# gnlpfjh/Scalable-E3-GNN

Measured on AMD Instinct MI355X. Metric: particles/sec (octree build + SEGNN fwd), 1M pts l_max=2, 1/2/4/8 MI355X, higher is better.
Workload: dtype f32; 1 GPU; 1000000 particles/GPU uniform in unit box, radius graph k~24 (E=23519616), SEGNN l_max=2 4 layers H=32 f32 storage; particles_per_gpu=1000000, edges_per_gpu=23519616, hidden=32, layers=4, lmax=2, parallelism=single GPU

## Files before the change

### scalable-e3-gnn_amd/csrc/e3_msg_ws.hip

```cpp
#include "e3_msg_plan.h"
#include "cg_tables.h"

#include <algorithm>
#include <type_traits>

#ifndef E3_WS_STAMP
#define E3_WS_STAMP 0
#endif

namespace e3 {
#include "e3_tp_mfma_core.h"
#include "e3_msg_common.h"

#if E3_WS_STAMP
__device__ unsigned long long g_ws_stamps[8][4];
__device__ unsigned long long g_ws_tp[8][8];
#define WS_TPMARK(i) { if (tpm) { const uint32_t t_ = (uint32_t)__builtin_readcyclecounter(); tpm[i] += t_ - tpm0; tpm0 = t_; } }
#define WS_TPPIN(v) asm volatile("" : "+v"(v));
#else
#define WS_TPMARK(i)
#define WS_TPPIN(v)
#endif

template <int LMAX, int TT, bool IO16>
struct Ws {
  using G = MsgGeom<LMAX, TT>;
  static_assert(TT == 2 && (LMAX == 1 || LMAX == 2), "instantiated for H = 32, l_max = 1 / 2");
  static constexpr int H = G::H, D = G::D, NS = G::NS, UD = G::UD;
  static constexpr int ES = IO16 ? 2 : 4;
  static constexpr int NC = (LMAX + 1) * (LMAX + 1);
  static constexpr int NFR = NC + LMAX;
  static constexpr int FRB = IO16 ? 1024 : 2048;
  static constexpr int frag(int l, int a) { return l * l + a; }
  static constexpr int frag_ff(int l) { return NC + l - 1; }
  static constexpr int GA_ROW = (NC - 1) * H * ES;
  static constexpr int GA_STRIDE = GA_ROW + 16;
  static constexpr int GA_BYTES = 16 * GA_STRIDE;
  static constexpr int GB_ROW = H * ES;
  static constexpr int GB_BYTES = 16 * GB_ROW;
  static constexpr int G_BYTES = GA_BYTES + GB_BYTES;
  static constexpr int RS = D + 4;
  static constexpr int U_ROW = UD * 4;
  static constexpr int U_PIECES = (U_ROW + 1023) / 1024, U_LAST = (U_ROW - (U_PIECES - 1) * 1024) / 16;
  static_assert(U_ROW % 16 == 0, "pre-mix rows are copied in 16-byte units");
  static constexpr int o_tab = 0;
  static constexpr int o_tinfo = (o_tab + (2 * NS * 16 + G::WD) * 4 + 15) / 16 * 16;
  static constexpr int o_ids = o_tinfo + 4 * 32;
  static constexpr int o_idok = o_ids + 4 * 128;
  static constexpr int o_pos = o_idok + 16;
  static constexpr int o_hmx = o_pos + 2 * 512;
  static constexpr int o_srow = o_hmx + 2 * 128;
  static constexpr int z_y = 0, z_112 = 12, z_121 = 28, z_211 = 40, z_222 = 56, ZT = LMAX == 2 ? 84 : 12;
  static constexpr int o_zt = o_srow + 2 * 64;
  static constexpr int o_init = o_zt + 2 * 16 * ZT * 4;
  static constexpr bool PRE = !IO16;
  static constexpr int P_AROW = (NC - 1) * 128;
  static constexpr int P_ASTRIDE = P_AROW + 32;
  static constexpr int P_ALANES = P_AROW / 16;
  static constexpr int o_pz = 16 * P_ASTRIDE, o_pf = o_pz + 2048;
  static constexpr int P_IMG = o_pf + LMAX * 2048;
  static constexpr int p_asrc(int lane) { return 128 + 16 * lane; }
  static constexpr int p_alds(int row, int lane) { return row * P_ASTRIDE + 16 * lane; }
  static constexpr int p_zrow(int piece, int lane) { return 8 * piece + (lane & 7); }
  static constexpr int p_zsrc(int lane) { return 64 * ((lane >> 5) & 1) + 16 * (2 * ((lane >> 4) & 1) + ((lane >> 3) & 1)); }
  static constexpr int p_zlds(int piece, int lane) { return o_pz + 1024 * piece + 16 * lane; }
  static constexpr int p_zpos(int lane) {
    return 1024 * ((lane & 15) >> 3) + 256 * (lane >> 5) + 128 * ((lane >> 4) & 1) + 16 * (lane & 7);
  }
  static constexpr int p_abase(int lane) { return (lane & 15) * P_ASTRIDE + 16 * (lane >> 4); }
  static constexpr int p_zbase(int lane) { return o_pz + p_zpos(lane); }
  static constexpr bool p_on_a(int fr) { return fr >= 1 && fr < NC; }
  static constexpr int p_off(int fr, int half) {
    return p_on_a(fr) ? 128 * (fr - 1) + 64 * half : (fr == 0 ? 0 : 2048 * (1 + fr - NC)) + 512 * half;
  }
  static constexpr int p_read(int fr, int half, int lane) { return (p_on_a(fr) ? p_abase(lane) : p_zbase(lane)) + p_off(fr, half); }
  static constexpr int o_g = o_init + G::T(0) * 1024;
  static constexpr int o_b1 = o_g + (PRE ? 2 * P_IMG : G_BYTES);
  static constexpr int o_b2 = o_b1 + (PRE ? 0 : NFR * FRB);
  static constexpr int o_o = o_b2 + NFR * FRB;
  static constexpr int o_u = o_o + 16 * RS * 4;
  static constexpr int total = o_u + 4 * U_ROW;
  static_assert(total <= 160 * 1024, "LDS image exceeds the CU");
};

template <int LMAX, int TT>
struct WsImageCheck {
  using L = Ws<LMAX, TT, false>;
  static constexpr int NU = L::o_pf / 16;
  static constexpr int group_lane(int grp, int i) {
    const int base = 32 * (grp >> 1), odd = grp & 1;
    const int k = odd ? (i < 8 ? 4 + i : (i < 12 ? 16 + (i - 8) : 28 + (i - 12))) : (i < 4 ? i : (i < 8 ? 12 + (i - 4) : 20 + (i - 8)));
    return base + k;
  }
  static constexpr bool run() {
    int owner_row[NU] = {}, owner_unit[NU] = {}, count[NU] = {};
    for (int r = 0; r < 16; ++r)
      for (int l = 0; l < L::P_ALANES; ++l) {
        const int u = L::p_alds(r, l) / 16;
        if (L::p_alds(r, l) % 16 || u < 0 || u >= NU) return false;
        ++count[u]; owner_row[u] = r; owner_unit[u] = L::p_asrc(l) / 16;
      }
    for (int p = 0; p < 2; ++p)
      for (int l = 0; l < 64; ++l) {
        const int u = L::p_zlds(p, l) / 16;
        if (u < 0 || u >= NU) return false;
        ++count[u]; owner_row[u] = L::p_zrow(p, l); owner_unit[u] = L::p_zsrc(l) / 16;
      }
    int written = 0;
    for (int u = 0; u < NU; ++u) {
      if (count[u] > 1) return false;
      written += count[u];
    }
    if (written != 16 * MsgSplit<LMAX>::UNITS) return false;
    for (int fr = 0; fr < L::NC; ++fr)
      for (int half = 0; half < 2; ++half) {
        for (int lane = 0; lane < 64; ++lane) {
          const int a = L::p_read(fr, half, lane), u = a / 16;
          if (a % 16 || u < 0 || u >= NU || count[u] != 1) return false;
          if (owner_row[u] != (lane & 15) || owner_unit[u] != MsgSplit<LMAX>::unit(fr, half, lane >> 4)) return false;
        }
      }
    for (int fr = 0; fr < L::NFR; ++fr)
      for (int half = 0; half < 2; ++half)
        for (int grp = 0; grp < 4; ++grp) {
          bool seen[16] = {};
          for (int i = 0; i < 16; ++i) {
            const int a = L::p_read(fr, half, group_lane(grp, i));
            if (a < 0 || a + 16 > L::P_IMG) return false;
            const int slot = (a % 256) / 16;
            if (seen[slot]) return false;
            seen[slot] = true;
          }
        }
    for (int fr = L::NC; fr < L::NFR; ++fr)
      for (int half = 0; half < 2; ++half)
        for (int lane = 0; lane < 64; ++lane)
          for (int l2 = lane + 1; l2 < 64; ++l2)
            if (L::p_read(fr, half, lane) == L::p_read(fr, half, l2) || L::p_read(fr, half, lane) < L::o_pf) return false;
    return true;
  }
};
static_assert(WsImageCheck<2, 2>::run() && WsImageCheck<1, 2>::run(), "pre-split image: coverage, read map or bank conflicts");

struct TileInfo { int e0, n, n0, node0, node1, sl0, sl1; };

__device__ __forceinline__ void dma16(const void* gsrc, uint32_t lds_dst) {
  uint32_t keep;
  asm volatile("s_mov_b32 %0, m0\n\ts_mov_b32 m0, %2\n\ts_nop 0\n\tglobal_load_lds_dwordx4 %1, off\n\ts_mov_b32 m0, %0"
               : "=&s"(keep) : "v"(gsrc), "s"(lds_dst) : "memory");
}
__device__ __forceinline__ void dma16_stream(const void* gsrc, uint32_t lds_dst) {
  uint32_t keep;
  asm volatile("s_mov_b32 %0, m0\n\ts_mov_b32 m0, %2\n\ts_nop 0\n\tglobal_load_lds_dwordx4 %1, off nt\n\ts_mov_b32 m0, %0"
               : "=&s"(keep) : "v"(gsrc), "s"(lds_dst) : "memory");
}
__device__ __forceinline__ void dma4(const void* gsrc, uint32_t lds_dst) {
  uint32_t keep;
  asm volatile("s_mov_b32 %0, m0\n\ts_mov_b32 m0, %2\n\ts_nop 0\n\tglobal_load_lds_dword %1, off\n\ts_mov_b32 m0, %0"
               : "=&s"(keep) : "v"(gsrc), "s"(lds_dst) : "memory");
}
__device__ __forceinline__ void ws_wait_vm0() { asm volatile("s_waitcnt vmcnt(0)" ::: "memory"); }
__device__ __forceinline__ void ws_barrier() { asm volatile("s_waitcnt lgkmcnt(0)\n\ts_barrier" ::: "memory"); }
__device__ __forceinline__ int sgpr(int v) { return __builtin_amdgcn_readfirstlane(v); }
__device__ __forceinline__ void split2_f16_scaled(const float v0, const float v1, const float s, uint32_t& hi, uint32_t& lo) {
  uint32_t h, l;
  asm("v_fma_mixlo_f16 %0, %1, %2, 0 op_sel_hi:[0,0,0]" : "=v"(h) : "v"(s), "v"(v0));
  asm("v_fma_mixhi_f16 %0, %1, %2, 0 op_sel_hi:[0,0,0]" : "+v"(h) : "v"(s), "v"(v1));
  asm("v_fma_mixlo_f16 %0, %1, %2, -%3 op_sel:[0,0,0] op_sel_hi:[0,0,1]" : "=v"(l) : "v"(s), "v"(v0), "v"(h));
  asm("v_fma_mixhi_f16 %0, %1, %2, -%3 op_sel:[0,0,1] op_sel_hi:[0,0,1]" : "+v"(l) : "v"(s), "v"(v1), "v"(h));
  hi = h; lo = l;
}
template <bool IO16>
__device__ __forceinline__ void ws_put4(unsigned char* dst, const float (&f)[4], const float s) {
  if constexpr (IO16) {
    const uint32_t a = __builtin_bit_cast(uint32_t, __builtin_convertvector(f32x2_t{f[0], f[1]}, bf16x2_t));
    const uint32_t b = __builtin_bit_cast(uint32_t, __builtin_convertvector(f32x2_t{f[2], f[3]}, bf16x2_t));
    *reinterpret_cast<uint2*>(dst) = uint2{a, b};
  } else {
    uint32_t h0, l0, h1, l1;
    split2_f16_scaled(f[0], f[1], s, h0, l0);
    split2_f16_scaled(f[2], f[3], s, h1, l1);
    *reinterpret_cast<uint2*>(dst) = uint2{h0, h1};
    *reinterpret_cast<uint2*>(dst + 1024) = uint2{l0, l1};
  }
}
template <int HI>
__device__ __forceinline__ float fma_mix_h(const float z, const uint32_t pair, const float acc) {
  float d;
  if constexpr (HI) asm("v_fma_mix_f32 %0, %1, %2, %3 op_sel:[0,1,0] op_sel_hi:[0,1,0]" : "=v"(d) : "v"(z), "v"(pair), "v"(acc));
  else asm("v_fma_mix_f32 %0, %1, %2, %3 op_sel:[0,0,0] op_sel_hi:[0,1,0]" : "=v"(d) : "v"(z), "v"(pair), "v"(acc));
  return d;
}
__device__ __forceinline__ uint32_t u4_word(const uint4& v, const int i) { return i == 0 ? v.x : i == 1 ? v.y : i == 2 ? v.z : v.w; }
template <class F>
__device__ __forceinline__ void sfor3(F&& f) {
  f(std::integral_constant<int, 0>{}); f(std::integral_constant<int, 1>{}); f(std::integral_constant<int, 2>{});
}

template <int LMAX, int TT, int ROLE>
struct Own {
  using G = MsgGeom<LMAX, TT>;
  static constexpr int t = ROLE & 1;
  static constexpr int LV = ROLE < 2 ? LMAX : LMAX - 1;
  static constexpr int tG = LV > 0 ? TT * LV + t : -1;
  static constexpr int tS = ROLE >= 2 ? t : -1;
  static constexpr int sl3(int s) { return s == 0 ? LV : 0; }
  static constexpr int stile(int s) { return s == 0 ? t : s == 1 ? tG : tS; }
  static constexpr bool shas(int s) { return s == 0 ? LV > 0 : stile(s) >= 0; }
  static constexpr bool has(int s, int l1, int l2) { return shas(s) && G::ok(l1, l2, sl3(s)); }
  static constexpr int widx(int s, int l1, int l2) {
    int n = 0;
    for (int ss = 0; ss < 3; ++ss)
      for (int a = 0; a <= LMAX; ++a)
        for (int b = 0; b <= LMAX; ++b) {
          if (ss == s && a == l1 && b == l2) return has(ss, a, b) ? n : -1;
          if (has(ss, a, b)) ++n;
        }
    return n;
  }
  static constexpr int NW = widx(3, 0, 0);
};

template <int NW>
struct RoleW { uint4 h[NW], l[NW]; };

template <int LMAX, int TT, int ROLE, bool IO16>
__device__ __forceinline__ void ws_load_w(const float* packed, const int prod , const int lane,
                                          RoleW<Own<LMAX, TT, ROLE>::NW>& w) {
  using G = MsgGeom<LMAX, TT>;
  using O = Own<LMAX, TT, ROLE>;
  const unsigned char* base = reinterpret_cast<const unsigned char*>(packed + G::o_w) + (size_t)prod * G::nblk() * 2048 + lane * 16;
  auto one = [&](auto stag, auto atag, auto btag) {
    constexpr int s = decltype(stag)::value, l1 = decltype(atag)::value, l2 = decltype(btag)::value;
    if constexpr (l1 <= LMAX && l2 <= LMAX && O::has(s, l1, l2)) {
      constexpr int i = O::widx(s, l1, l2), blk = G::blk(l1, l2, O::sl3(s)) + O::stile(s);
      w.h[i] = *reinterpret_cast<const uint4*>(base + (size_t)blk * 2048);
      if constexpr (!IO16) w.l[i] = *reinterpret_cast<const uint4*>(base + (size_t)blk * 2048 + 1024);
      else w.l[i] = uint4{0, 0, 0, 0};
    }
  };
  using I0 = std::integral_constant<int, 0>; using I1 = std::integral_constant<int, 1>; using I2 = std::integral_constant<int, 2>;
  auto slot = [&](auto stag) {
    one(stag, I0{}, I0{}); one(stag, I0{}, I1{}); one(stag, I0{}, I2{});
    one(stag, I1{}, I0{}); one(stag, I1{}, I1{}); one(stag, I1{}, I2{});
    one(stag, I2{}, I0{}); one(stag, I2{}, I1{}); one(stag, I2{}, I2{});
  };
  slot(I0{}); slot(I1{}); slot(I2{});
}

constexpr int kWsPF = 2;
constexpr int kWsXrot = 2;
constexpr int kWsPKT = 15;
#ifndef WS_PKZ
#define WS_PKZ 11
#endif
constexpr int kWsPrio = 0;
template <int LMAX>
struct TpItems {
  static constexpr int N = (LMAX + 1) * (LMAX + 1) + LMAX;
  static constexpr int len(int l) { return 2 * l + 1 + (l > 0 ? 1 : 0); }
  static constexpr int start(int l) { int n = 0; for (int k = LMAX; k > l; --k) n += len(k); return n; }
  static constexpr int l1(int i) { int l = LMAX; while (l > 0 && i >= start(l) + len(l)) --l; return l; }
  static constexpr int a(int i) { const int l = l1(i), k = i - start(l); return k < 2 * l + 1 ? k : -1; }
  static constexpr bool first(int i) { return i == start(l1(i)); }
};

template <int LMAX, int TT, int ROLE, bool FIRST, bool IO16>
struct TpRun {
  using G = MsgGeom<LMAX, TT>;
  using O = Own<LMAX, TT, ROLE>;
  using L = Ws<LMAX, TT, IO16>;
  using IT = TpItems<LMAX>;
  static constexpr int LV = O::LV, t = O::t, tG = O::tG, tS = O::tS;
  static constexpr bool SC = tG >= 0 || tS >= 0;

  static constexpr bool PIMG = FIRST && L::PRE;
  const RoleW<O::NW>& w;
  const unsigned char* bfr;
  const unsigned char* bfz;
  int lane;
  const float* zt;
  const float* urow;
  const float* wd;
  const f32x4* init;
  f32x4 (&accV)[5];
  f32x4& accG;
  f32x4& accS;
  float dsc;
  uint4 bh[kWsPF + 1], bl[kWsPF + 1];
  f32x4 uV[3][3][5];
  f32x4 wdV;
  f32x4 yv[3];
  f32x4 zq[3][3][7];
#if E3_WS_STAMP
  uint32_t* tpm = nullptr;
  uint32_t tpm0 = 0;
#endif
  static constexpr int zoff(int l1, int l2) {
    return (l1 == 1 && l2 == 1 && LV == 2) ? L::z_112 : (l1 == 1 && l2 == 2 && LV == 1) ? L::z_121
         : (l1 == 2 && l2 == 1 && LV == 1) ? L::z_211 : (l1 == 2 && l2 == 2 && LV == 2) ? L::z_222 : -1;
  }
  __device__ __forceinline__ float yy(const int i) const { return yv[i >> 2][i & 3]; }

  template <int I>
  __device__ __forceinline__ void request() {
    if constexpr (I < IT::N) {
      constexpr int L1 = IT::l1(I), a = IT::a(I), slot = I % (kWsPF + 1);
      constexpr int fr = a >= 0 ? L::frag(L1, a) : L::frag_ff(L1);
      if constexpr (a >= 0 || SC) {
        if constexpr (PIMG) {
          const unsigned char* b = bfr;
          if constexpr (!L::p_on_a(fr)) {
            int l = lane;
            asm volatile("" : "+v"(l));
            b = bfz + L::p_zbase(l);
          }
          bh[slot] = *reinterpret_cast<const uint4*>(b + L::p_off(fr, 0));
          bl[slot] = *reinterpret_cast<const uint4*>(b + L::p_off(fr, 1));
        } else {
          bh[slot] = *reinterpret_cast<const uint4*>(bfr + fr * L::FRB);
          if constexpr (!IO16) bl[slot] = *reinterpret_cast<const uint4*>(bfr + fr * L::FRB + 1024);
          else bl[slot] = uint4{0, 0, 0, 0};
        }
      }
      const f32x4 zero4 = {0.f, 0.f, 0.f, 0.f};
      if constexpr (a >= 0) {
        sfor3([&](auto l2tag) {
          constexpr int L2 = decltype(l2tag)::value;
          if constexpr (LV > 0 && G::ok(L1, L2, LV)) {
            if constexpr (FIRST) uV[L1][L2][a] = *reinterpret_cast<const f32x4*>(urow + G::uoff(L1, L2, LV) + (a * G::T(LV) + t) * 16);
            else uV[L1][L2][a] = zero4;
            if constexpr (a == 0 && zoff(L1, L2) >= 0) {
              constexpr int NZ = ((2 * L1 + 1) * (2 * LV + 1) + 3) / 4;
#pragma unroll
              for (int q = 0; q < NZ; ++q) zq[L1][L2][q] = *reinterpret_cast<const f32x4*>(zt + zoff(L1, L2) + 4 * q);
            }
          }
        });
        if constexpr (L1 == 0 && FIRST && LV > 0) wdV = *reinterpret_cast<const f32x4*>(wd + G::wdoff(LV) + t * 16);
      }
    }
  }

  template <int I>
  __device__ __forceinline__ void compute() {
    constexpr int L1 = IT::l1(I), a = IT::a(I), slot = I % (kWsPF + 1);
    const uint4 xh = bh[slot], xl = bl[slot];
    if constexpr (a >= 0) {
      if constexpr (L1 == 0 && FIRST && LV > 0) {
        uV[0][LV][0] = __builtin_elementwise_fma(wdV, f32x4{dsc, dsc, dsc, dsc}, uV[0][LV][0]);
      }
      sfor3([&](auto l2tag) {
        constexpr int L2 = decltype(l2tag)::value;
        if constexpr (LV > 0 && G::ok(L1, L2, LV)) {
          constexpr int i = O::widx(0, L1, L2);
          uV[L1][L2][a] = mma3<IO16>(w.h[i], w.l[i], xh, xl, uV[L1][L2][a]);
        }
      });
      if constexpr (L1 == 0) {
        if constexpr (tG >= 0) accG = mma3<IO16>(w.h[O::widx(1, 0, 0)], w.l[O::widx(1, 0, 0)], xh, xl, accG);
        if constexpr (tS >= 0) accS = mma3<IO16>(w.h[O::widx(2, 0, 0)], w.l[O::widx(2, 0, 0)], xh, xl, accS);
      }
    } else if constexpr (SC) {
      if constexpr (tG >= 0) accG = mma3<IO16>(w.h[O::widx(1, L1, L1)], w.l[O::widx(1, L1, L1)], xh, xl, accG);
      if constexpr (tS >= 0) accS = mma3<IO16>(w.h[O::widx(2, L1, L1)], w.l[O::widx(2, L1, L1)], xh, xl, accS);
    }
  }

  template <int L1>
  __device__ __forceinline__ void fold() {
    constexpr int D1 = 2 * L1 + 1;
    sfor3([&](auto l2tag) {
      constexpr int L2 = decltype(l2tag)::value;
      if constexpr (LV > 0 && G::ok(L1, L2, LV)) {
        constexpr int D3 = 2 * LV + 1;
        if constexpr (zoff(L1, L2) >= 0) {
#pragma unroll
          for (int c = 0; c < D3; ++c)
#pragma unroll
            for (int aa = 0; aa < D1; ++aa)
              if (z_nonzero<L1, L2, LV>(aa, c)) {
                const float z = zq[L1][L2][(aa * D3 + c) >> 2][(aa * D3 + c) & 3];
                constexpr int zi = (L1 == 1 && L2 == 1) ? 0 : (L1 == 1 && L2 == 2) ? 1 : (L1 == 2 && L2 == 1) ? 2 : 3;
                if constexpr (!IO16 && (kWsPKT & 1) && ((WS_PKZ >> zi) & 1)) {
                  accV[c] = __builtin_elementwise_fma(uV[L1][L2][aa], f32x4{z, z, z, z}, accV[c]);
                } else {
#pragma unroll
                  for (int r = 0; r < 4; ++r) accV[c][r] = __builtin_fmaf(uV[L1][L2][aa][r], z, accV[c][r]);
                }
              }
        } else {
          float y9[9];
#pragma unroll
          for (int i = 0; i < 9; ++i) y9[i] = yy(i);
          float zz[D1][D3];
          make_z<L1, L2, LV>(y9, zz);
#pragma unroll
          for (int c = 0; c < D3; ++c)
#pragma unroll
            for (int aa = 0; aa < D1; ++aa)
              if (z_nonzero<L1, L2, LV>(aa, c)) {
                if constexpr (!IO16 && (kWsPKT & 2)) {
                  accV[c] = __builtin_elementwise_fma(uV[L1][L2][aa], f32x4{zz[aa][c], zz[aa][c], zz[aa][c], zz[aa][c]}, accV[c]);
                } else {
#pragma unroll
                  for (int r = 0; r < 4; ++r) accV[c][r] = __builtin_fmaf(uV[L1][L2][aa][r], zz[aa][c], accV[c][r]);
                }
              }
        }
      }
    });
  }

  template <int I>
  __device__ __forceinline__ void step() {
    request<I + kWsPF>();
    __builtin_amdgcn_sched_barrier(0);
    compute<I>();
    if constexpr (IT::first(I) && IT::l1(I) < LMAX) fold<IT::l1(I) + 1>();
    if constexpr (I + 1 < IT::N && IT::first(I + 1)) { WS_TPMARK(1 + LMAX - IT::l1(I)) }
    if constexpr (I + 1 < IT::N) step<I + 1>();
    else { pin_products(); WS_TPMARK(1 + LMAX) fold<0>(); pin_folds(); WS_TPMARK(2 + LMAX) }
  }
  __device__ __forceinline__ void pin_products() {
    if constexpr (LV > 0) { WS_TPPIN(uV[0][LV][0]) }
    WS_TPPIN(accG) WS_TPPIN(accS)
  }
  __device__ __forceinline__ void pin_folds() {
#pragma unroll
    for (int c = 0; c < 2 * LV + 1; ++c) { WS_TPPIN(accV[c]) }
  }

  __device__ __forceinline__ void run() {
    const f32x4 zero4 = {0.f, 0.f, 0.f, 0.f};
#pragma unroll
    for (int c = 0; c < 5; ++c) accV[c] = zero4;
#pragma unroll
    for (int q = 0; q < 3; ++q) yv[q] = *reinterpret_cast<const f32x4*>(zt + L::z_y + 4 * q);
    accG = zero4; accS = zero4;
    if constexpr (FIRST) {
      if constexpr (tG >= 0) accG = init[64 * tG];
      if constexpr (tS >= 0) accS = init[64 * tS];
    }
    request<0>();
    if constexpr (kWsPF >= 2) request<1>();
    if constexpr (kWsPF >= 3) request<2>();
    static_assert(kWsPF >= 1 && kWsPF <= 3, "prefetch distance");
    __builtin_amdgcn_sched_barrier(0);
    dsc = yv[2][1];
    WS_TPMARK(0)
    step<0>();
  }
};

template <int LMAX, int TT, int ROLE, bool FIRST, bool IO16>
__device__ __forceinline__ void ws_tp(const RoleW<Own<LMAX, TT, ROLE>::NW>& w, const unsigned char* bfr,
                                      const unsigned char* bfz, const int lane, const float* zt,
                                      const float* urow, const float* wd, const f32x4* init,
                                      f32x4 (&accV)[5], f32x4& accG, f32x4& accS, float (&y)[10], uint32_t* tpmarks = nullptr) {
  TpRun<LMAX, TT, ROLE, FIRST, IO16> r{w, bfr, bfz, lane, zt, urow, wd, init, accV, accG, accS};
#if E3_WS_STAMP
  r.tpm = tpmarks;
  r.tpm0 = (uint32_t)__builtin_readcyclecounter();
#endif
  r.run();
#pragma unroll
  for (int i = 0; i < 10; ++i) y[i] = r.yy(i);
}

template <class BOX>
struct WsArgsT {
  const void* h; int64_t ldh;
  const float4* pos4; const int32_t* src; const int32_t* dst; int64_t E;
  const float* packed; const float* U; const void* split; const float* hmax; const float* in_scale; float* out; int64_t ldo;
  int chunk;
  float* part; int* part_node; uint32_t* amax; int chunks_per_xcd;
  BOX box;
};
using WsArgs = WsArgsT<PbcBox>;

template <int LMAX, int TT, bool IO16, int W, int PBC>
__device__ __forceinline__ void ws_run(const WsArgsT<typename PbcArg<PBC>::type>& A, unsigned char* smem) {
  using G = MsgGeom<LMAX, TT>;
  using L = Ws<LMAX, TT, IO16>;
  constexpr int H = G::H, D = G::D, ES = L::ES;
  constexpr bool TEAM1 = W >= 4;
  constexpr int ROLE = W & 3;
  constexpr int SX = TEAM1 ? -1 : ((W + kWsXrot) & 3);
  constexpr int ITB = SX < 0 ? 0 : L::PRE ? (SX == 2 ? 4 : 0) : 2 * SX;
  constexpr int ITE0 = SX < 0 ? 0 : L::PRE ? (SX == 1 ? 4 : (SX == 2 ? 6 : 0)) : (SX <= 2 ? 2 * SX + 2 : 2 * SX);
  constexpr int ITE = ITE0 < G::T(0) ? ITE0 : G::T(0);
  constexpr int SY = TEAM1 ? (W & 3) : -1;
  using O = Own<LMAX, TT, ROLE>;
  using I0 = std::integral_constant<int, 0>; using I1 = std::integral_constant<int, 1>; using I2 = std::integral_constant<int, 2>;
  const int lane = threadIdx.x & 63, j = lane & 15, g = lane >> 4;
  const uint32_t lds0 = (uint32_t)(uintptr_t)smem;
  const float* n1tab = reinterpret_cast<const float*>(smem + L::o_tab);
  const float* n2tab = n1tab + G::NS * 16;
  const float* wdtab = n2tab + G::NS * 16;
  const float xs = (!IO16 && A.in_scale) ? A.in_scale[0] : 1.0f;
  const float bwx = A.packed[6] * ((!IO16 && A.in_scale) ? A.in_scale[1] : 1.0f);
  const char* hb = reinterpret_cast<const char*>(A.h);

  auto tinfo = [&](const int tile) -> TileInfo {
    TileInfo ti = {0, 0, 0, -1, -1, 0, 0};
    if (tile >= 0) {
      const int4* p = reinterpret_cast<const int4*>(smem + L::o_tinfo + (tile & 3) * 32);
      const int4 a = p[0], b = p[1];
      ti.e0 = sgpr(a.x); ti.n = sgpr(a.y); ti.n0 = sgpr(a.z); ti.node0 = sgpr(a.w);
      ti.node1 = sgpr(b.x); ti.sl0 = sgpr(b.y); ti.sl1 = sgpr(b.z);
    }
    return ti;
  };

  RoleW<O::NW> w;
  ws_load_w<LMAX, TT, ROLE, IO16>(A.packed, TEAM1 ? 1 : 0, lane, w);
  wait_vm0();
  f32x4 nrS = {0.f, 0.f, 0.f, 0.f}, nrG = {0.f, 0.f, 0.f, 0.f}, nrV[5];
  {
    const f32x4* ntq = reinterpret_cast<const f32x4*>(TEAM1 ? n2tab : n1tab) + g;
    if constexpr (O::tS >= 0) nrS = ntq[4 * O::tS];
#pragma unroll
    for (int c = 0; c < 5; ++c) nrV[c] = f32x4{0.f, 0.f, 0.f, 0.f};
    if constexpr (O::LV > 0) {
      nrG = ntq[4 * O::tG];
#pragma unroll
      for (int c = 0; c < 2 * O::LV + 1; ++c) nrV[c] = ntq[4 * (G::slot0(O::LV) + (2 * O::LV + 1) * O::t + c)];
    }
  }

  const int Ei = (int)A.E;
  const int per_xcd = (int)(gridDim.x >> 3), wg_idx = (int)(blockIdx.x >> 3);
  const int e_per_xcd = ((Ei + 7) / 8 + 15) / 16 * 16;
  const int xlo = (int)(blockIdx.x & 7) * e_per_xcd;
  const int xhi = xlo + e_per_xcd < Ei ? xlo + e_per_xcd : Ei;

  auto gather_part = [&](const int tile, const int part) {
    const int* ids = reinterpret_cast<const int*>(smem + L::o_ids) + (tile & 3) * 32;
    if constexpr (L::PRE) {
      const uint32_t ib = lds0 + L::o_g + (tile & 1) * L::P_IMG;
      const char* sp = reinterpret_cast<const char*>(A.split);
      const int myid = ids[lane & 15];
      const int zid = ids[L::p_zrow(part, lane)];
      asm volatile("s_waitcnt lgkmcnt(0)" ::: "memory");
#pragma unroll
      for (int k = 0; k < 8; ++k) {
        const int r = 8 * part + k;
        const int rid = part == 0 ? __builtin_amdgcn_readlane(myid, k) : __builtin_amdgcn_readlane(myid, 8 + k);
        const char* rowp = sp + (int64_t)rid * MsgSplit<LMAX>::BYTES;
        if (L::P_ALANES >= 64 || lane < L::P_ALANES) dma16(rowp + L::p_asrc(lane), sgpr((int)(ib + L::p_alds(r, 0))));
// ... 232 lines not shown
        __builtin_amdgcn_sched_barrier(0);
        float y[9], dist;
        if constexpr (LMAX == 2) edge_sh<PBC>(ps, pd, y, dist, A.box); else edge_sh1<PBC>(ps, pd, y, dist, A.box);
        auto put4 = [&](const int fr, const float (&f)[4]) { ws_put4<IO16>(b1 + fr * L::FRB, f, xs); };
        auto degree = [&](auto ltag, float* q) {
          constexpr int L1 = decltype(ltag)::value, D1 = 2 * L1 + 1;
#pragma unroll
          for (int a = 0; a < D1; ++a) {
            const float f[4] = {q[a], q[D1 + a], q[2 * D1 + a], q[3 * D1 + a]};
            put4(L::frag(L1, a), f);
          }
          if constexpr (L1 > 0) {
            float zz[D1][1];
            make_z<L1, L1, 0>(y, zz);
            float f[4];
#pragma unroll
            for (int r = 0; r < 4; ++r) {
              float sum = zz[0][0] * q[r * D1];
#pragma unroll
              for (int a = 1; a < D1; ++a) sum = __builtin_fmaf(zz[a][0], q[r * D1 + a], sum);
              f[r] = sum;
            }
            put4(L::frag_ff(L1), f);
          }
        };
        if constexpr (LMAX == 2) degree(I2{}, q2);
        degree(I1{}, q1);
        degree(I0{}, q0);
      }
      if ((ITB < ITE || SX == 2) && t0.n > 0) {
        const float4* pp = reinterpret_cast<const float4*>(smem + L::o_pos + (s & 1) * 512);
        const float4 ps = pp[j], pd = pp[16 + j];
        const int slot = (j >= t0.n0 && j < t0.n) ? t0.sl1 : t0.sl0;
        const float* urow = reinterpret_cast<const float*>(smem + L::o_u + slot * L::U_ROW) + 4 * g;
        constexpr int T0 = G::T(0);
        float y[9], dist;
        if constexpr (LMAX == 2) edge_sh<PBC>(ps, pd, y, dist, A.box); else edge_sh1<PBC>(ps, pd, y, dist, A.box);
        const float dsc = dist * xs;
        if constexpr (SX == 2 && !IO16) {
          const float* hm = reinterpret_cast<const float*>(smem + L::o_hmx + (s & 1) * 128);
          const float srow = pow2_scale_from_bits(__builtin_bit_cast(uint32_t, bwx * fmaxf(fmaxf(hm[j], hm[16 + j]), dsc)), 12);
          if (lane < 16) reinterpret_cast<float*>(smem + L::o_srow)[(s & 1) * 16 + lane] = srow;
        }
        float z110[3][1], z220[5][1];
        make_z<1, 1, 0>(y, z110);
        if constexpr (LMAX == 2) make_z<2, 2, 0>(y, z220);
        f32x4* ip = reinterpret_cast<f32x4*>(smem + L::o_init) + lane;
        static_assert(T0 == 6 || T0 == 4, "two scalar-type tiles per wave (0, 1, 2 / 0, 1)");
#pragma unroll
        for (int t2 = ITB; t2 < ITE; t2 += 2) {
          f32x4 u0[2], u1[3][2], u2[5][2], wv[2];
#pragma unroll
          for (int k = 0; k < 2; ++k) {
            const int tt = t2 + k;
            u0[k] = *reinterpret_cast<const f32x4*>(urow + G::uoff(0, 0, 0) + tt * 16);
            wv[k] = *reinterpret_cast<const f32x4*>(wdtab + 4 * g + G::wdoff(0) + tt * 16);
#pragma unroll
            for (int a = 0; a < 3; ++a) u1[a][k] = *reinterpret_cast<const f32x4*>(urow + G::uoff(1, 1, 0) + (a * T0 + tt) * 16);
            if constexpr (LMAX == 2) {
#pragma unroll
              for (int a = 0; a < 5; ++a) u2[a][k] = *reinterpret_cast<const f32x4*>(urow + G::uoff(2, 2, 0) + (a * T0 + tt) * 16);
            }
          }
          __builtin_amdgcn_sched_barrier(0);
#pragma unroll
          for (int k = 0; k < 2; ++k) {
            f32x4 v = u0[k];
#pragma unroll
            for (int r = 0; r < 4; ++r) {
              v[r] = __builtin_fmaf(wv[k][r], dsc, v[r]);
#pragma unroll
              for (int a = 0; a < 3; ++a) v[r] = __builtin_fmaf(u1[a][k][r], z110[a][0], v[r]);
              if constexpr (LMAX == 2) {
#pragma unroll
                for (int a = 0; a < 5; ++a) v[r] = __builtin_fmaf(u2[a][k][r], z220[a][0], v[r]);
              }
            }
            ip[64 * (t2 + k)] = v;
          }
          __builtin_amdgcn_sched_barrier(0);
        }
        if constexpr (SX == 2) {
        float* zr = reinterpret_cast<float*>(smem + L::o_zt + (s & 1) * 16 * L::ZT * 4) + j * L::ZT;
        auto store_dense = [&](auto atag, auto btag, auto ctag, float* dstp) {
          constexpr int A1 = decltype(atag)::value, B1 = decltype(btag)::value, C1 = decltype(ctag)::value;
          constexpr int Da = 2 * A1 + 1, Dc = 2 * C1 + 1, NE = Da * Dc;
          float zz[Da][Dc];
          make_z<A1, B1, C1>(y, zz);
          float flat[(NE + 3) / 4 * 4];
#pragma unroll
          for (int i = 0; i < (NE + 3) / 4 * 4; ++i) flat[i] = i < NE ? zz[i / Dc][i % Dc] : 0.f;
#pragma unroll
          for (int q = 0; q < (NE + 3) / 4; ++q)
            *reinterpret_cast<f32x4*>(dstp + 4 * q) = f32x4{flat[4 * q], flat[4 * q + 1], flat[4 * q + 2], flat[4 * q + 3]};
        };
        if (g == 0) {
          *reinterpret_cast<f32x4*>(zr + L::z_y) = f32x4{y[0], y[1], y[2], y[3]};
          *reinterpret_cast<f32x4*>(zr + L::z_y + 4) = f32x4{y[4], y[5], y[6], y[7]};
          *reinterpret_cast<f32x4*>(zr + L::z_y + 8) = f32x4{y[8], dsc, 0.f, 0.f};
          if constexpr (LMAX == 2) store_dense(I1{}, I1{}, I2{}, zr + L::z_112);
        } else if constexpr (LMAX == 2) {
          if (g == 1) {
            store_dense(I1{}, I2{}, I1{}, zr + L::z_121);
          } else if (g == 2) {
            store_dense(I2{}, I1{}, I1{}, zr + L::z_211);
          } else {
            store_dense(I2{}, I2{}, I2{}, zr + L::z_222);
          }
        }
        }
      }
    } else {
      if (t1.n > 0) {
        float y[10];
        const float* ztr = reinterpret_cast<const float*>(smem + L::o_zt + ((s - 1) & 1) * 16 * L::ZT * 4) + j * L::ZT;
        const uint32_t sb = reinterpret_cast<const uint32_t*>(smem + L::o_srow)[((s - 1) & 1) * 16 + j];
        const float isrow = IO16 ? 1.0f : __builtin_bit_cast(float, 0x7F000000u - sb);
        f32x4 accV[5], accG, accS;
        __builtin_amdgcn_s_setprio(kWsPrio);
        WS_PM(5)
        ws_tp<LMAX, TT, ROLE, false, IO16>(w, smem + L::o_b2 + lane * 16, nullptr, lane, ztr, nullptr, nullptr, nullptr, accV, accG, accS, y, tpmk);
        WS_PM0
        [[maybe_unused]] const f32x4* nt = reinterpret_cast<const f32x4*>(n2tab) + g;
        float* orow = reinterpret_cast<float*>(smem + L::o_o) + j * L::RS;
        if constexpr (O::tS >= 0) {
          const f32x4 nv = nrS;
          f32x4 o;
#pragma unroll
          for (int r = 0; r < 4; ++r) {
            const float sv = accS[r] * nv[r] * isrow;
            o[r] = sv * sigmoid_(sv);
          }
          *reinterpret_cast<f32x4*>(orow + 16 * O::t + 4 * g) = o;
        }
        if constexpr (O::LV > 0) {
          constexpr int Dc = 2 * O::LV + 1;
          const f32x4 gn = nrG;
          f32x4 gt;
#pragma unroll
          for (int r = 0; r < 4; ++r) gt[r] = sigmoid_(accG[r] * gn[r] * isrow) * isrow;
          float o[4 * Dc];
#pragma unroll
          for (int c = 0; c < Dc; ++c) {
            const f32x4 nv = nrV[c];
            f32x4 oc;
            if constexpr (!IO16 && (kWsPKT & 4)) {
              oc = accV[c] * nv * gt;
            } else {
#pragma unroll
              for (int r = 0; r < 4; ++r) oc[r] = accV[c][r] * nv[r] * gt[r];
            }
#pragma unroll
            for (int r = 0; r < 4; ++r) o[r * Dc + c] = oc[r];
          }
          f32x4* dq = reinterpret_cast<f32x4*>(orow + G::col0(O::LV) + (16 * O::t + 4 * g) * Dc);
#pragma unroll
          for (int k = 0; k < Dc; ++k) dq[k] = f32x4{o[4 * k], o[4 * k + 1], o[4 * k + 2], o[4 * k + 3]};
        }
      }
    }
    if constexpr (TEAM1) __builtin_amdgcn_s_setprio(0);
    WS_PM(6)
    WS_STAMP(0)
    ws_barrier();
    WS_STAMP(1)
    WS_PM0
    if constexpr (!TEAM1) {
      if (t0.n > 0) {
        float y[10];
        const float* ztr = reinterpret_cast<const float*>(smem + L::o_zt + (s & 1) * 16 * L::ZT * 4) + j * L::ZT;
        float srow = 1.0f;
        if constexpr (!IO16) srow = reinterpret_cast<const float*>(smem + L::o_srow)[(s & 1) * 16 + j];
        const int slot = (j >= t0.n0 && j < t0.n) ? t0.sl1 : t0.sl0;
        const float* urow = reinterpret_cast<const float*>(smem + L::o_u + slot * L::U_ROW) + 4 * g;
        f32x4 accV[5], accG, accS;
        __builtin_amdgcn_s_setprio(kWsPrio);
        WS_PM(5)
        const unsigned char* img = smem + L::o_g + (L::PRE ? (s & 1) * L::P_IMG : 0);
        ws_tp<LMAX, TT, ROLE, true, IO16>(w, L::PRE ? img + L::p_abase(lane) : smem + L::o_b1 + lane * 16,
                                          L::PRE ? img : nullptr, lane, ztr, urow, wdtab + 4 * g,
                                          reinterpret_cast<const f32x4*>(smem + L::o_init) + lane, accV, accG, accS, y, tpmk);
        WS_PM0
        [[maybe_unused]] const f32x4* nt = reinterpret_cast<const f32x4*>(n1tab) + g;
        unsigned char* b2 = smem + L::o_b2 + lane * 16 + 8 * O::t;
        auto put4 = [&](const int fr, const float (&f)[4]) { ws_put4<IO16>(b2 + fr * L::FRB, f, srow); };
        if constexpr (O::tS >= 0) {
          const f32x4 nv = nrS;
          float f[4];
#pragma unroll
          for (int r = 0; r < 4; ++r) {
            const float sv = accS[r] * nv[r];
            f[r] = sv * sigmoid_(sv);
          }
          put4(L::frag(0, 0), f);
        }
        if constexpr (O::LV > 0) {
          constexpr int Dc = 2 * O::LV + 1;
          const f32x4 gn = nrG;
          f32x4 gt;
#pragma unroll
          for (int r = 0; r < 4; ++r) gt[r] = sigmoid_(accG[r] * gn[r]);
          float y9[9];
#pragma unroll
          for (int i = 0; i < 9; ++i) y9[i] = y[i];
          float zz[Dc][1];
          make_z<O::LV, O::LV, 0>(y9, zz);
          f32x4 fsv = {0.f, 0.f, 0.f, 0.f};
#pragma unroll
          for (int c = 0; c < Dc; ++c) {
            const f32x4 nv = nrV[c];
            f32x4 fv;
            if constexpr (!IO16 && (kWsPKT & 8)) {
              fv = accV[c] * nv * gt;
              const f32x4 zc = {zz[c][0], zz[c][0], zz[c][0], zz[c][0]};
              fsv = c == 0 ? zc * fv : __builtin_elementwise_fma(zc, fv, fsv);
            } else {
#pragma unroll
              for (int r = 0; r < 4; ++r) {
                fv[r] = accV[c][r] * nv[r] * gt[r];
                fsv[r] = c == 0 ? zz[0][0] * fv[r] : __builtin_fmaf(zz[c][0], fv[r], fsv[r]);
              }
            }
            const float f[4] = {fv[0], fv[1], fv[2], fv[3]};
            put4(L::frag(O::LV, c), f);
          }
          const float fs[4] = {fsv[0], fsv[1], fsv[2], fsv[3]};
          put4(L::frag_ff(O::LV), fs);
        }
      }
      if constexpr (SX == 3) ws_wait_vm0();
    } else if constexpr (RSW) {
      if (t1.n > 0) {
        const float* op = reinterpret_cast<const float*>(smem + L::o_o) + lane;
        float s0[NQW], s1[NQW];
#pragma unroll
        for (int q = 0; q < NQW; ++q) { s0[q] = 0.f; s1[q] = 0.f; }
        float v[16][NQW];
#pragma unroll
        for (int r = 0; r < 16; ++r)
#pragma unroll
          for (int q = 0; q < Q1 - Q0; ++q) v[r][q] = (64 * (Q0 + q) + lane < D) ? op[r * L::RS + 64 * (Q0 + q)] : 0.f;
        __builtin_amdgcn_sched_barrier(0);
        if (t1.n0 == 16) {
#pragma unroll
          for (int r = 0; r < 16; ++r)
#pragma unroll
            for (int q = 0; q < Q1 - Q0; ++q) s0[q] += v[r][q];
        } else {
#pragma unroll
          for (int r = 0; r < 16; ++r) {
#pragma unroll
            for (int q = 0; q < Q1 - Q0; ++q) {
              s0[q] += r < t1.n0 ? v[r][q] : 0.f;
              s1[q] += (r >= t1.n0 && r < t1.n) ? v[r][q] : 0.f;
            }
          }
        }
        const bool cstart = owned && t1.e0 == onext;
        if (cstart || t1.node0 != cur) {
          flush(cstart);
          if (cstart) { ocur = ochunk; onfl = 0; ochunk += per_xcd; onext += per_xcd * A.chunk; }
          cur = t1.node0;
        }
#pragma unroll
// ... 147 lines not shown
```

Baseline: 12.06 million particles/s.

## Pack CG coupling table to nonzero entries and reorder table reads per role

Replaces the dense per-edge Clebsch-Gordan coefficient table in LDS with a packed layout that stores only the structurally nonzero entries, grouped per role degree into two aligned blocks. Each role now reads only its own block into a flat register array, with part of the reads deferred into the pipeline. The srow load and the z-base pointer computation move into the tensor-product runner, and the issue of B-fragment requests is moved ahead of the table reads. This is meant to cut LDS footprint, LDS read traffic and register pressure, at the cost of more complex unaligned store sequences. WS_PKZ also changes from 11 to 10, which turns off the packed-FMA path for one coupling path.

```diff
diff --git a/scalable-e3-gnn_amd/csrc/e3_msg_ws.hip b/scalable-e3-gnn_amd/csrc/e3_msg_ws.hip
--- a/scalable-e3-gnn_amd/csrc/e3_msg_ws.hip
+++ b/scalable-e3-gnn_amd/csrc/e3_msg_ws.hip
@@ -21,6 +21,24 @@
 #define WS_TPMARK(i)
 #define WS_TPPIN(v)
 #endif
+
+template <int L1, int L2, int L3>
+struct ZPack {
+  static constexpr int D1 = 2 * L1 + 1, D3 = 2 * L3 + 1;
+  struct Tab { int r[D1 * D3 + 1]; };
+  static constexpr Tab make() {
+    Tab t{};
+    int n = 0;
+    for (int i = 0; i < D1 * D3; ++i) {
+      t.r[i] = n;
+      n += z_nonzero<L1, L2, L3>(i / D3, i % D3) ? 1 : 0;
+    }
+    t.r[D1 * D3] = n;
+    return t;
+  }
+  static constexpr Tab tab = make();
+  static constexpr int N = tab.r[D1 * D3];
+};
 
 template <int LMAX, int TT, bool IO16>
 struct Ws {
@@ -50,7 +68,15 @@
   static constexpr int o_pos = o_idok + 16;
   static constexpr int o_hmx = o_pos + 2 * 512;
   static constexpr int o_srow = o_hmx + 2 * 128;
-  static constexpr int z_y = 0, z_112 = 12, z_121 = 28, z_211 = 40, z_222 = 56, ZT = LMAX == 2 ? 84 : 12;
+  static constexpr int z_a = 0, z_b = LMAX == 2 ? 44 : 0;
+  static constexpr int z_ny(int lv) { return lv > 0 ? 2 * lv + 2 : 0; }
+  static constexpr int z_n(int lv) {
+    return z_ny(lv) + (LMAX == 2 ? (lv == 2 ? ZPack<2, 2, 2>::N + ZPack<1, 1, 2>::N : ZPack<2, 1, 1>::N + ZPack<1, 2, 1>::N) : 0);
+  }
+  static constexpr int ZT = LMAX == 2 ? 76 : 12;
+  static_assert(z_a % 4 == 0 && z_b % 4 == 0 && ZT % 4 == 0 && (ZT / 4) % 2 == 1 && z_n(LMAX) % 4 == 0 && z_n(LMAX - 1) % 4 == 0 &&
+                z_a + z_n(LMAX) + 1 <= (LMAX == 2 ? z_b : ZT) && z_b + z_n(LMAX - 1) + 1 <= ZT,
+                "table row: 16-byte aligned groups of whole vectors that do not overlap; odd row stride in 16-byte units");
   static constexpr int o_zt = o_srow + 2 * 64;
   static constexpr int o_init = o_zt + 2 * 16 * ZT * 4;
   static constexpr bool PRE = !IO16;
@@ -195,6 +221,19 @@
 template <class F>
 __device__ __forceinline__ void sfor3(F&& f) {
   f(std::integral_constant<int, 0>{}); f(std::integral_constant<int, 1>{}); f(std::integral_constant<int, 2>{});
+}
+template <int OFF, int NE>
+__device__ __forceinline__ void ws_store_run(float* row, const float (&v)[NE]) {
+  constexpr int P1 = (OFF % 2 == 1 && NE >= 1) ? 1 : 0;
+  constexpr int P2 = P1 + (((OFF + P1) % 4 == 2 && P1 + 2 <= NE) ? 2 : 0);
+  constexpr int P3 = P2 + (NE - P2) / 4 * 4;
+  constexpr int P4 = P3 + (NE - P3 >= 2 ? 2 : 0);
+  if constexpr (P1 == 1) row[OFF] = v[0];
+  if constexpr (P2 > P1) *reinterpret_cast<f32x2_t*>(row + OFF + P1) = f32x2_t{v[P1], v[P1 + 1]};
+#pragma unroll
+  for (int p = P2; p < P3; p += 4) *reinterpret_cast<f32x4*>(row + OFF + p) = f32x4{v[p], v[p + 1], v[p + 2], v[p + 3]};
+  if constexpr (P4 > P3) *reinterpret_cast<f32x2_t*>(row + OFF + P3) = f32x2_t{v[P3], v[P3 + 1]};
+  if constexpr (P4 < NE) row[OFF + P4] = v[P4];
 }
 
 template <int LMAX, int TT, int ROLE>
@@ -252,7 +291,7 @@
 constexpr int kWsXrot = 2;
 constexpr int kWsPKT = 15;
 #ifndef WS_PKZ
-#define WS_PKZ 11
+#define WS_PKZ 10
 #endif
 constexpr int kWsPrio = 0;
 template <int LMAX>
@@ -278,8 +317,8 @@
   const RoleW<O::NW>& w;
   const unsigned char* bfr;
   const unsigned char* bfz;
-  int lane;
   const float* zt;
+  const float* srowp;
   const float* urow;
   const float* wd;
   const f32x4* init;
@@ -287,20 +326,34 @@
   f32x4& accG;
   f32x4& accS;
   float dsc;
+  float srow;
   uint4 bh[kWsPF + 1], bl[kWsPF + 1];
   f32x4 uV[3][3][5];
   f32x4 wdV;
-  f32x4 yv[3];
-  f32x4 zq[3][3][7];
+  static constexpr int ZB = LV == LMAX ? L::z_a : L::z_b, ZY = L::z_ny(LV), ZN = L::z_n(LV);
+  float zf[ZN + 1];
 #if E3_WS_STAMP
   uint32_t* tpm = nullptr;
   uint32_t tpm0 = 0;
 #endif
   static constexpr int zoff(int l1, int l2) {
-    return (l1 == 1 && l2 == 1 && LV == 2) ? L::z_112 : (l1 == 1 && l2 == 2 && LV == 1) ? L::z_121
-         : (l1 == 2 && l2 == 1 && LV == 1) ? L::z_211 : (l1 == 2 && l2 == 2 && LV == 2) ? L::z_222 : -1;
-  }
-  __device__ __forceinline__ float yy(const int i) const { return yv[i >> 2][i & 3]; }
+    return (l1 == 2 && l2 == 2 && LV == 2) ? ZY : (l1 == 1 && l2 == 1 && LV == 2) ? ZY + ZPack<2, 2, 2>::N
+         : (l1 == 2 && l2 == 1 && LV == 1) ? ZY : (l1 == 1 && l2 == 2 && LV == 1) ? ZY + ZPack<2, 1, 1>::N : -1;
+  }
+  static constexpr int ZH = (LMAX == 2 && LV > 0) ? (ZY + ZPack<LMAX, LV == LMAX ? LMAX : 1, LV>::N + 3) / 4 * 4 : ZN;
+  static_assert(ZN % 4 == 0 && ZH <= ZN, "whole vectors");
+  template <int LO, int HI>
+  __device__ __forceinline__ void zread() {
+    static_assert(LO % 4 == 0 && HI % 4 == 0, "pieces start and end on read boundaries");
+#pragma unroll
+    for (int p = LO; p < HI; p += 4) {
+      const f32x4 v = *reinterpret_cast<const f32x4*>(zt + ZB + p);
+      zf[p] = v[0]; zf[p + 1] = v[1]; zf[p + 2] = v[2]; zf[p + 3] = v[3];
+    }
+  }
+  __device__ __forceinline__ float yy(const int i) const {
+    return i == 0 ? zf[0] : (LV > 0 && i >= LV * LV && i < (LV + 1) * (LV + 1)) ? zf[1 + i - LV * LV] : 0.f;
+  }
 
   template <int I>
   __device__ __forceinline__ void request() {
@@ -309,12 +362,7 @@
       constexpr int fr = a >= 0 ? L::frag(L1, a) : L::frag_ff(L1);
       if constexpr (a >= 0 || SC) {
         if constexpr (PIMG) {
-          const unsigned char* b = bfr;
-          if constexpr (!L::p_on_a(fr)) {
-            int l = lane;
-            asm volatile("" : "+v"(l));
-            b = bfz + L::p_zbase(l);
-          }
+          const unsigned char* b = L::p_on_a(fr) ? bfr : bfz;
           bh[slot] = *reinterpret_cast<const uint4*>(b + L::p_off(fr, 0));
           bl[slot] = *reinterpret_cast<const uint4*>(b + L::p_off(fr, 1));
         } else {
@@ -330,13 +378,9 @@
           if constexpr (LV > 0 && G::ok(L1, L2, LV)) {
             if constexpr (FIRST) uV[L1][L2][a] = *reinterpret_cast<const f32x4*>(urow + G::uoff(L1, L2, LV) + (a * G::T(LV) + t) * 16);
             else uV[L1][L2][a] = zero4;
-            if constexpr (a == 0 && zoff(L1, L2) >= 0) {
-              constexpr int NZ = ((2 * L1 + 1) * (2 * LV + 1) + 3) / 4;
-#pragma unroll
-              for (int q = 0; q < NZ; ++q) zq[L1][L2][q] = *reinterpret_cast<const f32x4*>(zt + zoff(L1, L2) + 4 * q);
-            }
           }
         });
+        if constexpr (LMAX >= 2 && I == IT::start(LMAX - 1) && ZH < ZN) zread<ZH, ZN>();
         if constexpr (L1 == 0 && FIRST && LV > 0) wdV = *reinterpret_cast<const f32x4*>(wd + G::wdoff(LV) + t * 16);
       }
     }
@@ -380,7 +424,7 @@
 #pragma unroll
             for (int aa = 0; aa < D1; ++aa)
               if (z_nonzero<L1, L2, LV>(aa, c)) {
-                const float z = zq[L1][L2][(aa * D3 + c) >> 2][(aa * D3 + c) & 3];
+                const float z = zf[zoff(L1, L2) + ZPack<L1, L2, LV>::tab.r[aa * D3 + c]];
                 constexpr int zi = (L1 == 1 && L2 == 1) ? 0 : (L1 == 1 && L2 == 2) ? 1 : (L1 == 2 && L2 == 1) ? 2 : 3;
                 if constexpr (!IO16 && (kWsPKT & 1) && ((WS_PKZ >> zi) & 1)) {
                   accV[c] = __builtin_elementwise_fma(uV[L1][L2][aa], f32x4{z, z, z, z}, accV[c]);
@@ -390,6 +434,7 @@
                 }
               }
         } else {
+          static_assert(L2 == 0 || L2 == LV, "the role's table group holds y0 and the harmonics of degree LV");
           float y9[9];
 #pragma unroll
           for (int i = 0; i < 9; ++i) y9[i] = yy(i);
@@ -435,19 +480,21 @@
     const f32x4 zero4 = {0.f, 0.f, 0.f, 0.f};
 #pragma unroll
     for (int c = 0; c < 5; ++c) accV[c] = zero4;
-#pragma unroll
-    for (int q = 0; q < 3; ++q) yv[q] = *reinterpret_cast<const f32x4*>(zt + L::z_y + 4 * q);
+    request<0>();
+    if constexpr (kWsPF >= 2) request<1>();
+    if constexpr (kWsPF >= 3) request<2>();
+    static_assert(kWsPF >= 1 && kWsPF <= 3, "prefetch distance");
+    zread<0, ZH>();
+    if constexpr (FIRST) zf[ZN] = zt[ZB + ZN];
     accG = zero4; accS = zero4;
     if constexpr (FIRST) {
       if constexpr (tG >= 0) accG = init[64 * tG];
       if constexpr (tS >= 0) accS = init[64 * tS];
     }
-    request<0>();
-    if constexpr (kWsPF >= 2) request<1>();
-    if constexpr (kWsPF >= 3) request<2>();
-    static_assert(kWsPF >= 1 && kWsPF <= 3, "prefetch distance");
+    srow = 1.0f;
+    if constexpr (!IO16) srow = *srowp;
     __builtin_amdgcn_sched_barrier(0);
-    dsc = yv[2][1];
+    dsc = FIRST ? zf[ZN] : 0.f;
     WS_TPMARK(0)
     step<0>();
   }
@@ -455,17 +502,20 @@
 
 template <int LMAX, int TT, int ROLE, bool FIRST, bool IO16>
 __device__ __forceinline__ void ws_tp(const RoleW<Own<LMAX, TT, ROLE>::NW>& w, const unsigned char* bfr,
-                                      const unsigned char* bfz, const int lane, const float* zt,
+                                      const unsigned char* bfz, const float* zt, const float* srowp,
                                       const float* urow, const float* wd, const f32x4* init,
-                                      f32x4 (&accV)[5], f32x4& accG, f32x4& accS, float (&y)[10], uint32_t* tpmarks = nullptr) {
-  TpRun<LMAX, TT, ROLE, FIRST, IO16> r{w, bfr, bfz, lane, zt, urow, wd, init, accV, accG, accS};
+                                      f32x4 (&accV)[5], f32x4& accG, f32x4& accS, float (&y)[10], float& srow,
+                                      uint32_t* tpmarks = nullptr) {
+  TpRun<LMAX, TT, ROLE, FIRST, IO16> r{w, bfr, bfz, zt, srowp, urow, wd, init, accV, accG, accS};
 #if E3_WS_STAMP
   r.tpm = tpmarks;
   r.tpm0 = (uint32_t)__builtin_readcyclecounter();
 #endif
   r.run();
 #pragma unroll
-  for (int i = 0; i < 10; ++i) y[i] = r.yy(i);
+  for (int i = 0; i < 9; ++i) y[i] = r.yy(i);
+  y[9] = r.dsc;
+  srow = r.srow;
 }
 
 template <class BOX>
@@ -864,31 +914,38 @@
         }
         if constexpr (SX == 2) {
         float* zr = reinterpret_cast<float*>(smem + L::o_zt + (s & 1) * 16 * L::ZT * 4) + j * L::ZT;
-        auto store_dense = [&](auto atag, auto btag, auto ctag, float* dstp) {
+        auto store_dense = [&](auto atag, auto btag, auto ctag, auto offtag) {
           constexpr int A1 = decltype(atag)::value, B1 = decltype(btag)::value, C1 = decltype(ctag)::value;
           constexpr int Da = 2 * A1 + 1, Dc = 2 * C1 + 1, NE = Da * Dc;
+          using ZP = ZPack<A1, B1, C1>;
           float zz[Da][Dc];
           make_z<A1, B1, C1>(y, zz);
-          float flat[(NE + 3) / 4 * 4];
-#pragma unroll
-          for (int i = 0; i < (NE + 3) / 4 * 4; ++i) flat[i] = i < NE ? zz[i / Dc][i % Dc] : 0.f;
-#pragma unroll
-          for (int q = 0; q < (NE + 3) / 4; ++q)
-            *reinterpret_cast<f32x4*>(dstp + 4 * q) = f32x4{flat[4 * q], flat[4 * q + 1], flat[4 * q + 2], flat[4 * q + 3]};
+          float flat[ZP::N];
+#pragma unroll
+          for (int i = 0; i < NE; ++i)
+            if (z_nonzero<A1, B1, C1>(i / Dc, i % Dc)) flat[ZP::tab.r[i]] = zz[i / Dc][i % Dc];
+          ws_store_run<decltype(offtag)::value, ZP::N>(zr, flat);
         };
-        if (g == 0) {
-          *reinterpret_cast<f32x4*>(zr + L::z_y) = f32x4{y[0], y[1], y[2], y[3]};
-          *reinterpret_cast<f32x4*>(zr + L::z_y + 4) = f32x4{y[4], y[5], y[6], y[7]};
-          *reinterpret_cast<f32x4*>(zr + L::z_y + 8) = f32x4{y[8], dsc, 0.f, 0.f};
-          if constexpr (LMAX == 2) store_dense(I1{}, I1{}, I2{}, zr + L::z_112);
-        } else if constexpr (LMAX == 2) {
-          if (g == 1) {
-            store_dense(I1{}, I2{}, I1{}, zr + L::z_121);
+        const float y1d[4] = {y[0], y[1], y[2], y[3]}, dd[1] = {dsc};
+        if constexpr (LMAX == 2) {
+          constexpr int NA = L::z_n(2), NB = L::z_n(1), YA = L::z_ny(2), YB = L::z_ny(1);
+          if (g == 0) {
+            const float y2d[6] = {y[0], y[4], y[5], y[6], y[7], y[8]};
+            ws_store_run<L::z_a, 6>(zr, y2d);
+            store_dense(I1{}, I1{}, I2{}, std::integral_constant<int, L::z_a + YA + ZPack<2, 2, 2>::N>{});
+            ws_store_run<L::z_a + NA, 1>(zr, dd);
+          } else if (g == 1) {
+            ws_store_run<L::z_b, 4>(zr, y1d);
+            store_dense(I1{}, I2{}, I1{}, std::integral_constant<int, L::z_b + YB + ZPack<2, 1, 1>::N>{});
+            ws_store_run<L::z_b + NB, 1>(zr, dd);
           } else if (g == 2) {
-            store_dense(I2{}, I1{}, I1{}, zr + L::z_211);
+            store_dense(I2{}, I1{}, I1{}, std::integral_constant<int, L::z_b + YB>{});
           } else {
-            store_dense(I2{}, I2{}, I2{}, zr + L::z_222);
-          }
+            store_dense(I2{}, I2{}, I2{}, std::integral_constant<int, L::z_a + YA>{});
+          }
+        } else if (g == 0) {
+          ws_store_run<L::z_a, 4>(zr, y1d);
+          ws_store_run<L::z_a + L::z_n(1), 1>(zr, dd);
         }
         }
       }
@@ -896,13 +953,15 @@
       if (t1.n > 0) {
         float y[10];
         const float* ztr = reinterpret_cast<const float*>(smem + L::o_zt + ((s - 1) & 1) * 16 * L::ZT * 4) + j * L::ZT;
-        const uint32_t sb = reinterpret_cast<const uint32_t*>(smem + L::o_srow)[((s - 1) & 1) * 16 + j];
-        const float isrow = IO16 ? 1.0f : __builtin_bit_cast(float, 0x7F000000u - sb);
+        float srow;
         f32x4 accV[5], accG, accS;
         __builtin_amdgcn_s_setprio(kWsPrio);
         WS_PM(5)
-        ws_tp<LMAX, TT, ROLE, false, IO16>(w, smem + L::o_b2 + lane * 16, nullptr, lane, ztr, nullptr, nullptr, nullptr, accV, accG, accS, y, tpmk);
+        ws_tp<LMAX, TT, ROLE, false, IO16>(w, smem + L::o_b2 + lane * 16, nullptr, ztr,
+                                           reinterpret_cast<const float*>(smem + L::o_srow) + ((s - 1) & 1) * 16 + j, nullptr, nullptr,
+                                           nullptr, accV, accG, accS, y, srow, tpmk);
         WS_PM0
+        const float isrow = IO16 ? 1.0f : __builtin_bit_cast(float, 0x7F000000u - __builtin_bit_cast(uint32_t, srow));
         [[maybe_unused]] const f32x4* nt = reinterpret_cast<const f32x4*>(n2tab) + g;
         float* orow = reinterpret_cast<float*>(smem + L::o_o) + j * L::RS;
         if constexpr (O::tS >= 0) {
@@ -951,8 +1010,7 @@
       if (t0.n > 0) {
         float y[10];
         const float* ztr = reinterpret_cast<const float*>(smem + L::o_zt + (s & 1) * 16 * L::ZT * 4) + j * L::ZT;
-        float srow = 1.0f;
-        if constexpr (!IO16) srow = reinterpret_cast<const float*>(smem + L::o_srow)[(s & 1) * 16 + j];
+        float srow;
         const int slot = (j >= t0.n0 && j < t0.n) ? t0.sl1 : t0.sl0;
         const float* urow = reinterpret_cast<const float*>(smem + L::o_u + slot * L::U_ROW) + 4 * g;
         f32x4 accV[5], accG, accS;
@@ -960,8 +1018,9 @@
         WS_PM(5)
         const unsigned char* img = smem + L::o_g + (L::PRE ? (s & 1) * L::P_IMG : 0);
         ws_tp<LMAX, TT, ROLE, true, IO16>(w, L::PRE ? img + L::p_abase(lane) : smem + L::o_b1 + lane * 16,
-                                          L::PRE ? img : nullptr, lane, ztr, urow, wdtab + 4 * g,
-                                          reinterpret_cast<const f32x4*>(smem + L::o_init) + lane, accV, accG, accS, y, tpmk);
+                                          L::PRE ? img + L::p_zbase(lane) : nullptr, ztr,
+                                          reinterpret_cast<const float*>(smem + L::o_srow) + (s & 1) * 16 + j, urow, wdtab + 4 * g,
+                                          reinterpret_cast<const f32x4*>(smem + L::o_init) + lane, accV, accG, accS, y, srow, tpmk);
         WS_PM0
         [[maybe_unused]] const f32x4* nt = reinterpret_cast<const f32x4*>(n1tab) + g;
         unsigned char* b2 = smem + L::o_b2 + lane * 16 + 8 * O::t;
```

Result: no change. 12.14 million particles/s (median of 6 runs) (+0.6%).
